# MDFahimAnjum/AliasFree-Diffusion-Models-PyTorch

Hardware: AMD Instinct MI355X
Metric: train_step_images_per_sec (higher is better)
Workload: dtype f32; 1 GPU; CIFAR-10 32x32x3 synthetic, UNet variant=3 (Config D), batch 256/GPU, T=1000, AdamW lr 3e-4, random-init weights (seed 42); global_batch=256, parallelism=dp1, hip_graph=True, launch_mode=lanes

## Files before the change

### aliasfree-diffusion-models-pytorch_amd/_lib.py

```python
import ctypes
import os
import re

_PKG = os.path.dirname(os.path.abspath(__file__))
_ROOT = os.path.dirname(_PKG)
HEADER = os.path.join(_ROOT, "include", "afd.h")
LIBPATH = os.environ.get("AFD_LIBPATH") or os.path.join(_PKG, "libafd_hip.so")

_CTYPES = {
    "int": ctypes.c_int, "long": ctypes.c_long, "float": ctypes.c_float, "double": ctypes.c_double,
    "size_t": ctypes.c_size_t,
}
_DECL = re.compile(r"^(int|size_t|const char\*)\s+(afd_\w+)\s*\(([^;]*?)\)\s*;", re.M | re.S)


def _strip_comments(src):
    return re.sub(r"/\*.*?\*/", " ", src, flags=re.S)


def parse_header(path=HEADER):
    out = {}
    for ret, name, args in _DECL.findall(_strip_comments(open(path).read())):
        argtypes = []
        args = " ".join(args.split())
        if args not in ("", "void"):
            for a in args.split(","):
                a = a.strip()
                if "*" in a or a.startswith("afd_stream_t"):
                    argtypes.append(ctypes.c_void_p)
                else:
                    base = a.split()[0] if not a.startswith("unsigned") else a
                    argtypes.append(_CTYPES[base])
        restype = {"int": ctypes.c_int, "size_t": ctypes.c_size_t, "const char*": ctypes.c_char_p}[ret]
        out[name] = (restype, argtypes)
    return out


_VALUE_RETURNING = {"afd_device_count", "afd_tok_supported", "afd_conv3x3_weight_kinds", "afd_conv_wgrad_form", "afd_conv_wgrad3_plan",
                    "afd_grad_sqnorm_n_partials", "afd_debug_conv_state"}


class AfdError(RuntimeError):
    pass


class _Lib:
    def __init__(self):
        if not os.path.exists(LIBPATH):
            raise AfdError(
                f"{LIBPATH} not found: build it with `python -c 'import __graft_entry__ as g; g.build()'` "
                "(hipcc --offload-arch=gfx950). There is no CPU/eager fallback.")
        self.cdll = ctypes.CDLL(LIBPATH)
        self.sigs = parse_header()
        for name, (restype, argtypes) in self.sigs.items():
# ... 28 lines not shown
```

### aliasfree-diffusion-models-pytorch_amd/csrc/tok.hip

```cpp
#include "tok_common.h"
#include "tok_h2.h"
#include <algorithm>
#include <cstdint>
#include <mutex>
#include <set>

namespace afd {

template <int KB>
__device__ __forceinline__ f32x16 t_block(const float* __restrict__ Ws, int nb, int l31, int half, const TT<KB>& z, f32x16 acc) {
  constexpr int WS = 32 * KB + 4;
  const float* __restrict__ wr = Ws + (nb * 32 + l31) * WS + 4 * half;
#pragma unroll
  for (int j = 0; j < KB; ++j)
#pragma unroll
    for (int q = 0; q < 4; ++q) {
      const float4 a = *reinterpret_cast<const float4*>(wr + 32 * j + 8 * q);
      acc = __builtin_amdgcn_mfma_f32_32x32x2f32(a.x, z.b[j][4 * q + 0], acc, 0, 0, 0);
      acc = __builtin_amdgcn_mfma_f32_32x32x2f32(a.y, z.b[j][4 * q + 1], acc, 0, 0, 0);
      acc = __builtin_amdgcn_mfma_f32_32x32x2f32(a.z, z.b[j][4 * q + 2], acc, 0, 0, 0);
      acc = __builtin_amdgcn_mfma_f32_32x32x2f32(a.w, z.b[j][4 * q + 3], acc, 0, 0, 0);
    }
  return acc;
}
// ... 639 lines not shown
static int g_tok_max_wg = 0;
static int g_tok_path = 0;
static bool use_h2(int C, long ntile, int kern) {
  if (C != 64 && C != 128) return false;
  if (g_tok_path >= 4) return true;
  if (g_tok_path != 0) return false;
  if (C == 64) return ntile >= 1024 || (kern == 2 && ntile >= 512);
  return kern != 1 && ntile >= 512;
}
static bool use_wide(int C, long ntile) {
  if (C != 64 && C != 128) return false;
  if (g_tok_max_wg > 0 || g_tok_path == 1) return false;
  if (g_tok_path == 2) return true;
  return C == 128 || ntile < 1024;
}
static unsigned chain_grid(int C, long ntile) {
  const long wg = (ntile + 3) / 4;
  const long cap = g_tok_max_wg > 0 ? g_tok_max_wg : (C > 64 ? 8192 : 1024);
  return (unsigned)std::min<long>(wg, cap);
}

}

using namespace afd;

extern "C" {

int afd_tok_supported(int C) { return tok_ok(C) ? 1 : 0; }
int afd_debug_tok_grid(int max_workgroups) { g_tok_max_wg = max_workgroups; return AFD_OK; }
int afd_debug_tok_path(int mode) {
  AFD_REQUIRE(mode >= 0 && mode <= 6, "afd_debug_tok_path: mode %d not in 0..6", mode);
  g_tok_path = mode;
  tok_h2_debug_tpw(mode == 5 ? 2 : (mode == 6 ? 4 : 0));
  return AFD_OK;
}

int afd_tok_head_fwd(const float* x, const float* gamma, const float* beta, const float* w, const float* bias, float* h_out,
                     float* stats_out, float* qkv, int B, int C, int P, float eps, afd_stream_t st) {
  AFD_REQUIRE(x && gamma && beta && w && qkv && B > 0 && P > 0, "afd_tok_head_fwd: NULL pointer or empty shape");
  AFD_REQUIRE(tok_ok(C), "afd_tok_head_fwd: C=%d not covered (32, 64, 128)", C);
  AFD_REQUIRE((long)B * P * 3 * C < (1L << 31), "afd_tok_head_fwd: tensor too large for 32-bit offsets");
  const int N = 3 * C;
  const long ntile = ((long)B * P + 31) / 32, wg_tiles = (ntile + 3) / 4;
  if (use_h2(C, ntile, 0)) return tok_h2_head_fwd(x, gamma, beta, w, bias, h_out, stats_out, qkv, B, C, P, eps, g_tok_max_wg, as_stream(st));
  if (use_wide(C, ntile) && aligned16(w) && (ntile <= 256 || g_tok_path == 2)) {
    const long waves = ntile * (N / 32);
    const dim3 wgrid((unsigned)((waves + 3) / 4));
    hipStream_t s = as_stream(st);
    if (C == 64) hipLaunchKernelGGL((tok_head_fwd_wide<64, 1>), wgrid, dim3(256), 0, s, x, gamma, beta, w, bias, h_out, stats_out, qkv, B, P, eps);
    else         hipLaunchKernelGGL((tok_head_fwd_wide<128, 1>), wgrid, dim3(256), 0, s, x, gamma, beta, w, bias, h_out, stats_out, qkv, B, P, eps);
    return check_launch("afd_tok_head_fwd");
  }
  int npw = 32;
  for (int cand : {N, 192, 128, 96, 64, 32}) {
    if (cand > N || N % cand != 0) continue;
    if (sizeof(float) * ((size_t)cand * (C + 5) + 2 * C) > 64 * 1024) continue;
    npw = cand;
    if (wg_tiles * (N / cand) >= 256) break;
  }
  const size_t lds = sizeof(float) * ((size_t)npw * (C + 5) + 2 * C);
// ... 6 lines not shown
  }
  return check_launch("afd_tok_head_fwd");
}

int afd_tok_tail_fwd(const float* att, const float* x, const float* wo, const float* bo, const float* gamma, const float* beta,
                     const float* w1, const float* b1, const float* w2, const float* b2, float* a_out, float* stats_out,
                     float* f_out, float* u_out, float* g_out, float* out, int B, int C, int P, float eps, afd_stream_t st) {
  AFD_REQUIRE(att && x && wo && bo && gamma && beta && w1 && b1 && w2 && b2 && out && B > 0 && P > 0,
              "afd_tok_tail_fwd: NULL pointer or empty shape");
  AFD_REQUIRE(tok_ok(C), "afd_tok_tail_fwd: C=%d not covered (32, 64, 128)", C);
  AFD_REQUIRE((long)B * P * C < (1L << 31), "afd_tok_tail_fwd: tensor too large for 32-bit offsets");
  const bool train = a_out != nullptr;
  AFD_REQUIRE(!train || (stats_out && f_out && u_out && g_out), "afd_tok_tail_fwd: a_out given but a saved-tensor pointer is NULL");
  const long ntile = ((long)B * P + 31) / 32;
  hipStream_t s = as_stream(st);
  if (use_h2(C, ntile, 1))
    return tok_h2_tail_fwd(att, x, wo, bo, gamma, beta, w1, b1, w2, b2, a_out, stats_out, f_out, u_out, g_out, out, B, C, P, eps, g_tok_max_wg, s);
  if (use_wide(C, ntile) && aligned16(wo) && aligned16(w1) && aligned16(w2)) {
    const dim3 wgrid((unsigned)((ntile + Wide<64>::TPW - 1) / Wide<64>::TPW)), wgrid128((unsigned)ntile);
#define AFD_TAILW(C_, T_, G_) hipLaunchKernelGGL((tok_tail_fwd_wide<C_, T_>), G_, dim3(256), 0, s, att, x, wo, bo, gamma, beta, w1, b1, w2, b2, \
                                                  a_out, stats_out, f_out, u_out, g_out, out, B, P, eps)
    if (C == 64) { if (train) AFD_TAILW(64, true, wgrid); else AFD_TAILW(64, false, wgrid); }
    else         { if (train) AFD_TAILW(128, true, wgrid128); else AFD_TAILW(128, false, wgrid128); }
#undef AFD_TAILW
    return check_launch("afd_tok_tail_fwd");
  }
  const size_t lds = chain_lds(C, 5);
  const dim3 grid(chain_grid(C, ntile));
#define AFD_TAIL(C_, T_) do { if (int rc = set_lds(tok_tail_fwd<C_, T_>, lds)) return rc; \
    hipLaunchKernelGGL((tok_tail_fwd<C_, T_>), grid, dim3(256), lds, s, att, x, wo, bo, gamma, beta, w1, b1, w2, b2, a_out, stats_out, \
                       f_out, u_out, g_out, out, B, P, eps); } while (0)
  switch (C) {
    case 32:  if (train) AFD_TAIL(32, true); else AFD_TAIL(32, false); break;
// ... 1 lines not shown
    default:  if (train) AFD_TAIL(128, true); else AFD_TAIL(128, false); break;
  }
#undef AFD_TAIL
  return check_launch("afd_tok_tail_fwd");
}

int afd_tok_tail_bwd(const float* d_out, const float* u, const float* a, const float* stats, const float* gamma, const float* w2,
                     const float* w1, const float* wo, float* du_out, float* df_out, float* da_out, float* datt_out, int B, int C,
                     int P, afd_stream_t st) {
  AFD_REQUIRE(d_out && u && a && stats && gamma && w2 && w1 && wo && du_out && df_out && da_out && datt_out && B > 0 && P > 0,
              "afd_tok_tail_bwd: NULL pointer or empty shape");
  AFD_REQUIRE(tok_ok(C), "afd_tok_tail_bwd: C=%d not covered (32, 64, 128)", C);
  AFD_REQUIRE((long)B * P * C < (1L << 31), "afd_tok_tail_bwd: tensor too large for 32-bit offsets");
  const long ntile = ((long)B * P + 31) / 32;
  hipStream_t s = as_stream(st);
  if (use_h2(C, ntile, 2)) return tok_h2_tail_bwd(d_out, u, a, stats, gamma, w2, w1, wo, du_out, df_out, da_out, datt_out, B, C, P, g_tok_max_wg, s);
  if (use_wide(C, ntile)) {
    if (C == 64) hipLaunchKernelGGL(tok_tail_bwd_wide<64>, dim3((unsigned)((ntile + 1) / 2)), dim3(256), 0, s, d_out, u, a, stats, gamma, w2, w1, wo, du_out, df_out, da_out, datt_out, B, P);
    else         hipLaunchKernelGGL(tok_tail_bwd_wide<128>, dim3((unsigned)ntile), dim3(256), 0, s, d_out, u, a, stats, gamma, w2, w1, wo, du_out, df_out, da_out, datt_out, B, P);
    return check_launch("afd_tok_tail_bwd");
  }
  const size_t lds = chain_lds(C, 1);
  const dim3 grid(chain_grid(C, ntile));
#define AFD_TB(C_) do { if (int rc = set_lds(tok_tail_bwd<C_>, lds)) return rc; \
    hipLaunchKernelGGL(tok_tail_bwd<C_>, grid, dim3(256), lds, s, d_out, u, a, stats, gamma, w2, w1, wo, du_out, df_out, da_out, datt_out, B, P); } while (0)
  switch (C) { case 32: AFD_TB(32); break; case 64: AFD_TB(64); break; default: AFD_TB(128); break; }
#undef AFD_TB
  return check_launch("afd_tok_tail_bwd");
}

int afd_tok_head_bwd(const float* dqkv, const float* x, const float* stats, const float* gamma, const float* w_in,
                     const float* d_res, float* dh_out, float* dx_out, int B, int C, int P, afd_stream_t st) {
  AFD_REQUIRE(dqkv && x && stats && gamma && w_in && d_res && dx_out && B > 0 && P > 0, "afd_tok_head_bwd: NULL pointer or empty shape");
  AFD_REQUIRE(tok_ok(C), "afd_tok_head_bwd: C=%d not covered (32, 64, 128)", C);
  AFD_REQUIRE((long)B * P * 3 * C < (1L << 31), "afd_tok_head_bwd: tensor too large for 32-bit offsets");
  const long ntile = ((long)B * P + 31) / 32;
  hipStream_t s = as_stream(st);
  if (use_h2(C, ntile, 3)) return tok_h2_head_bwd(dqkv, x, stats, gamma, w_in, d_res, dh_out, dx_out, B, C, P, g_tok_max_wg, s);
  if (use_wide(C, ntile)) {
    if (C == 64) hipLaunchKernelGGL(tok_head_bwd_wide<64>, dim3((unsigned)((ntile + 1) / 2)), dim3(256), 0, s, dqkv, x, stats, gamma, w_in, d_res, dh_out, dx_out, B, P);
    else         hipLaunchKernelGGL(tok_head_bwd_wide<128>, dim3((unsigned)ntile), dim3(256), 0, s, dqkv, x, stats, gamma, w_in, d_res, dh_out, dx_out, B, P);
    return check_launch("afd_tok_head_bwd");
  }
  const size_t lds = chain_lds(C, 1);
  const dim3 grid(chain_grid(C, ntile));
#define AFD_HB(C_) do { if (int rc = set_lds(tok_head_bwd<C_>, lds)) return rc; \
    hipLaunchKernelGGL(tok_head_bwd<C_>, grid, dim3(256), lds, s, dqkv, x, stats, gamma, w_in, d_res, dh_out, dx_out, B, P); } while (0)
  switch (C) { case 32: AFD_HB(32); break; case 64: AFD_HB(64); break; default: AFD_HB(128); break; }
#undef AFD_HB
  return check_launch("afd_tok_head_bwd");
}

}
```

### aliasfree-diffusion-models-pytorch_amd/csrc/tok_h2.hip

```cpp
#include "tok_common.h"
#include "h2_common.h"
#include "tok_h2.h"
#include <algorithm>

namespace afd {

template <int NB>
__device__ __forceinline__ void h_load(TT<NB>& z, const float* __restrict__ src, unsigned base, int P) {
#pragma unroll
  for (int j = 0; j < NB; ++j)
#pragma unroll
    for (int r = 0; r < 16; ++r) z.b[j][r] = (src + (size_t)tch(j, r) * P)[base];
}
template <int NB>
__device__ __forceinline__ void h_store(const TT<NB>& z, float* __restrict__ dst, unsigned base, int P, bool live) {
  if (!live) return;
#pragma unroll
  for (int j = 0; j < NB; ++j)
#pragma unroll
    for (int r = 0; r < 16; ++r) (dst + (size_t)tch(j, r) * P)[base] = z.b[j][r];
}

template <int KB> struct HP { h8 a[2 * KB], b[2 * KB]; };

template <int KB>
__device__ __forceinline__ float hp_split(const TT<KB>& z, HP<KB>& p) {
  float m = 0.f;
#pragma unroll
  for (int j = 0; j < KB; ++j)
#pragma unroll
    for (int r = 0; r < 16; ++r) m = fmaxf(m, fabsf(z.b[j][r]));
  m = fmaxf(m, __shfl_xor(m, 32, 64));
  const float s = h2_scale_for(m);
#pragma unroll
  for (int k = 0; k < 2 * KB; ++k) {
    float x[8];
// ... 6 lines not shown

template <int KB>
__device__ __forceinline__ f32x16 hp_block(const h8* __restrict__ img, int nb, int l31, int half, const HP<KB>& z) {
  constexpr int C = 32 * KB, NG = C / 8;
  const h8* __restrict__ w0 = img + half * C + nb * 32 + l31;
  const h8* __restrict__ w1 = w0 + NG * C;
  f32x16 acc = zero16();
#pragma unroll
  for (int k = 0; k < 2 * KB; ++k) {
    const h8 a1 = w0[2 * k * C], a2 = w1[2 * k * C];
    acc = __builtin_amdgcn_mfma_f32_32x32x16_f16(a2, z.a[k], acc, 0, 0, 0);
    acc = __builtin_amdgcn_mfma_f32_32x32x16_f16(a1, z.b[k], acc, 0, 0, 0);
    acc = __builtin_amdgcn_mfma_f32_32x32x16_f16(a1, z.a[k], acc, 0, 0, 0);
  }
  return acc;
}

template <int C> struct H2Lds {
  static constexpr int NG = C / 8, REC = 2 * NG * C;
  static constexpr bool RELOAD = C > 64;
  static constexpr int NSLOT = RELOAD ? 2 : 3;
  h8* img[3];
  float* winv[3];
  unsigned* rmax[3];
  float* vec;
  __device__ __forceinline__ void init(unsigned char* base) {
    h8* i0 = reinterpret_cast<h8*>(base);
    float* w0 = reinterpret_cast<float*>(i0 + NSLOT * REC);
    unsigned* r0 = reinterpret_cast<unsigned*>(w0 + NSLOT * C);
#pragma unroll
    for (int m = 0; m < 3; ++m) {
      const int s = m % NSLOT;
      img[m] = i0 + s * REC; winv[m] = w0 + s * C; rmax[m] = r0 + s * C;
    }
    vec = reinterpret_cast<float*>(r0 + NSLOT * C);
  }
  static size_t bytes(int nvec) { return (size_t)NSLOT * REC * 16 + (size_t)NSLOT * C * 8 + (size_t)nvec * C * 4; }
};

struct WSrc { const float* w; int ldw, n0, k0; };

template <int C, int NT> struct Stg {
  static constexpr int NG = C / 8, NR = C * NG / NT;
  float x[NR][8];
  static __device__ __forceinline__ void rec(int r, bool transposed, int& n, int& G) {
    const int i = (int)threadIdx.x + r * NT;
    if (transposed) { n = i % C; G = i / C; }
    else {
      const int lo = i & 63, hi = i >> 6;
      n = (hi % (C / 8)) * 8 + (lo & 7);
      G = (hi / (C / 8)) * 8 + (lo >> 3);
    }
  }
  __device__ __forceinline__ void load(const WSrc& q, bool transposed) {
#pragma unroll
    for (int r = 0; r < NR; ++r) {
      int n, G;
      rec(r, transposed, n, G);
      const int kb = 16 * (G >> 1) + 4 * (G & 1);
#pragma unroll
      for (int e = 0; e < 8; ++e) {
        const int k = kb + 8 * (e >> 2) + (e & 3);
        x[r][e] = transposed ? q.w[(long)(q.k0 + k) * q.ldw + q.n0 + n] : q.w[(long)(q.n0 + n) * q.ldw + q.k0 + k];
      }
    }
  }
  __device__ __forceinline__ void maxima(unsigned* __restrict__ rmax, bool transposed) const {
#pragma unroll
    for (int r = 0; r < NR; ++r) {
      int n, G;
      rec(r, transposed, n, G);
      float m = 0.f;
#pragma unroll
      for (int e = 0; e < 8; ++e) m = fmaxf(m, fabsf(x[r][e]));
      atomicMax(&rmax[n], __float_as_uint(m));
    }
  }
  __device__ __forceinline__ void store(h8* __restrict__ img, float* __restrict__ winv, const unsigned* __restrict__ rmax,
                                        bool transposed) const {
#pragma unroll
    for (int r = 0; r < NR; ++r) {
      int n, G;
      rec(r, transposed, n, G);
      const float sc = h2_scale_for(__uint_as_float(rmax[n]));
      h8 p0, p1;
      h2_split8(x[r], sc, p0, p1);
      img[G * C + n] = p0;
      img[(NG + G) * C + n] = p1;
      if (G == 0) winv[n] = h2_inv_pow2(sc);
    }
  }
};

template <int C, int NT, int M0, int CNT>
__device__ __forceinline__ void h2_stage(const H2Lds<C>& L, const WSrc* src, bool transposed) {
  Stg<C, NT> st[CNT];
#pragma unroll
  for (int i = 0; i < CNT; ++i) st[i].load(src[i], transposed);
#pragma unroll
  for (int i = 0; i < CNT; ++i)
    for (int c = threadIdx.x; c < C; c += NT) L.rmax[M0 + i][c] = 0u;
  __syncthreads();
#pragma unroll
  for (int i = 0; i < CNT; ++i) st[i].maxima(L.rmax[M0 + i], transposed);
  __syncthreads();
#pragma unroll
  for (int i = 0; i < CNT; ++i) st[i].store(L.img[M0 + i], L.winv[M0 + i], L.rmax[M0 + i], transposed);
  __builtin_amdgcn_sched_barrier(0);
}
template <int C, int NT>
__device__ __forceinline__ void h2_stage_first(const H2Lds<C>& L, const WSrc* src, bool transposed) {
  if (H2Lds<C>::RELOAD) h2_stage<C, NT, 0, 2>(L, src, transposed);
  else h2_stage<C, NT, 0, 3>(L, src, transposed);
}
template <int C, int NT, int M>
__device__ __forceinline__ void h2_stage_one(const H2Lds<C>& L, const WSrc* src, bool transposed) {
  h2_stage<C, NT, M, 1>(L, src + M, transposed);
}

struct Walk { int lane, wv, half, l31, ntile, tstride, t0, npass; unsigned total; };
template <int TPW> __device__ __forceinline__ Walk walk_of(int B, int P) {
  Walk k;
  k.lane = threadIdx.x & 63; k.wv = threadIdx.x >> 6; k.half = k.lane >> 5; k.l31 = k.lane & 31;
  k.total = (unsigned)B * (unsigned)P;
  k.ntile = (int)((k.total + 31u) / 32u);
  k.tstride = gridDim.x * TPW;
  k.t0 = blockIdx.x * TPW;
  k.npass = k.t0 < k.ntile ? (k.ntile - k.t0 + k.tstride - 1) / k.tstride : 0;
  return k;
}

extern __shared__ __attribute__((aligned(16))) unsigned char h2_smem[];
// ... 352 lines not shown
```

### include/afd.h

```cpp
#ifndef AFD_H_
#define AFD_H_

#include <stddef.h>
#include <stdint.h>

#ifdef __cplusplus
extern "C" {
#endif

#define AFD_OK 0
#define AFD_EINVAL 1
#define AFD_ELAUNCH 2
#define AFD_MAX_TAPS 15

typedef void* afd_stream_t;

const char* afd_version(void);
const char* afd_last_error(void);
int afd_device_count(void);

int afd_lowpass_kernel(double omega_c, int N, int has_beta, double beta, float* taps_out);

int afd_filt_up2_fwd(const float* x, float* y, int B, int C, int H, int W, long x_bstride, long y_bstride,
                     const float* taps, int N, afd_stream_t stream);
// ... 88 lines not shown
                        afd_stream_t stream);
int afd_layernorm_c_bwd_params(const float* x, const float* dy, const float* stats, int B, int C, int HW,
                               float* dgamma_dbeta_partial , float* dgamma, float* dbeta, int accumulate,
                               afd_stream_t stream);
int afd_layernorm_c_bwd_partials(const float* x, const float* dy, const float* stats, int B, int C, int HW, float* part,
                                 afd_stream_t stream);

int afd_debug_attn_rows(int rows);
int afd_attn_fwd(const float* qkv, float* o, float* lse, int B, int heads, int d, int L, afd_stream_t stream);
int afd_attn_bwd(const float* qkv, const float* o, const float* d_o, const float* lse, float* dqkv,
                 float* delta_workspace , int B, int heads, int d, int L, afd_stream_t stream);

int afd_tok_supported(int C);
int afd_debug_tok_grid(int max_workgroups);
int afd_debug_tok_path(int mode);
int afd_tok_head_fwd(const float* x, const float* gamma, const float* beta, const float* w_in, const float* b_in,
                     float* h_out, float* stats_out, float* qkv, int B, int C, int P, float eps, afd_stream_t stream);
int afd_tok_tail_fwd(const float* att, const float* x, const float* w_o, const float* b_o, const float* gamma, const float* beta,
                     const float* w_1, const float* b_1, const float* w_2, const float* b_2,
                     float* a_out, float* stats_out, float* f_out, float* u_out, float* g_out, float* out,
                     int B, int C, int P, float eps, afd_stream_t stream);
int afd_tok_tail_bwd(const float* d_out, const float* u, const float* a, const float* stats, const float* gamma,
                     const float* w_2, const float* w_1, const float* w_o,
                     float* du_out, float* df_out, float* da_out, float* datt_out, int B, int C, int P, afd_stream_t stream);
int afd_tok_head_bwd(const float* dqkv, const float* x, const float* stats, const float* gamma, const float* w_in,
                     const float* d_res, float* dh_out, float* dx_out, int B, int C, int P, afd_stream_t stream);

int afd_gelu_fwd(const float* x, float* y, long n, afd_stream_t stream);
int afd_gelu_bwd(const float* x, const float* dy, float* dx, long n, afd_stream_t stream);
int afd_maxpool2_fwd(const float* x, float* y, int B, int C, int H, int W, afd_stream_t stream);
// ... 299 lines not shown
```

Baseline: 39740 images/s.

## Add wide split-half tokenizer kernels for mid-size attention token counts

```diff
diff --git a/aliasfree-diffusion-models-pytorch_amd/_lib.py b/aliasfree-diffusion-models-pytorch_amd/_lib.py
--- a/aliasfree-diffusion-models-pytorch_amd/_lib.py
+++ b/aliasfree-diffusion-models-pytorch_amd/_lib.py
@@ -37,7 +37,7 @@
 
 
 _VALUE_RETURNING = {"afd_device_count", "afd_tok_supported", "afd_conv3x3_weight_kinds", "afd_conv_wgrad_form", "afd_conv_wgrad3_plan",
-                    "afd_grad_sqnorm_n_partials", "afd_debug_conv_state"}
+                    "afd_grad_sqnorm_n_partials", "afd_debug_conv_state", "afd_debug_tok_form"}
 
 
 class AfdError(RuntimeError):
diff --git a/aliasfree-diffusion-models-pytorch_amd/csrc/tok.hip b/aliasfree-diffusion-models-pytorch_amd/csrc/tok.hip
--- a/aliasfree-diffusion-models-pytorch_amd/csrc/tok.hip
+++ b/aliasfree-diffusion-models-pytorch_amd/csrc/tok.hip
@@ -1,5 +1,6 @@
 #include "tok_common.h"
 #include "tok_h2.h"
+#include "tok_h2w.h"
 #include <algorithm>
 #include <cstdint>
 #include <mutex>
@@ -677,6 +678,19 @@
   if (g_tok_path == 2) return true;
   return C == 128 || ntile < 1024;
 }
+static bool use_h2w(int C, long ntile, int kern) {
+  if (C != 64 && C != 128) return false;
+  if (g_tok_path == 7) return true;
+  if (g_tok_path != 0) return false;
+  if (C == 64) return ntile >= 512 && ntile < 1024 && kern != 1;
+  return ntile >= 128 && ntile < 512 && kern >= 2;
+}
+static int tok_form(int C, long ntile, int kern) {
+  if (use_h2w(C, ntile, kern)) return 3;
+  if (use_h2(C, ntile, kern)) return 2;
+  if (use_wide(C, ntile) && (kern != 0 || ntile <= 256 || g_tok_path == 2)) return 1;
+  return 0;
+}
 static unsigned chain_grid(int C, long ntile) {
   const long wg = (ntile + 3) / 4;
   const long cap = g_tok_max_wg > 0 ? g_tok_max_wg : (C > 64 ? 8192 : 1024);
@@ -692,10 +706,14 @@
 int afd_tok_supported(int C) { return tok_ok(C) ? 1 : 0; }
 int afd_debug_tok_grid(int max_workgroups) { g_tok_max_wg = max_workgroups; return AFD_OK; }
 int afd_debug_tok_path(int mode) {
-  AFD_REQUIRE(mode >= 0 && mode <= 6, "afd_debug_tok_path: mode %d not in 0..6", mode);
+  AFD_REQUIRE(mode >= 0 && mode <= 7, "afd_debug_tok_path: mode %d not in 0..7", mode);
   g_tok_path = mode;
   tok_h2_debug_tpw(mode == 5 ? 2 : (mode == 6 ? 4 : 0));
   return AFD_OK;
+}
+int afd_debug_tok_form(int C, int B, int P, int kern) {
+  if (!tok_ok(C) || B <= 0 || P <= 0 || kern < 0 || kern > 3) return -1;
+  return tok_form(C, ((long)B * P + 31) / 32, kern);
 }
 
 int afd_tok_head_fwd(const float* x, const float* gamma, const float* beta, const float* w, const float* bias, float* h_out,
@@ -705,8 +723,10 @@
   AFD_REQUIRE((long)B * P * 3 * C < (1L << 31), "afd_tok_head_fwd: tensor too large for 32-bit offsets");
   const int N = 3 * C;
   const long ntile = ((long)B * P + 31) / 32, wg_tiles = (ntile + 3) / 4;
-  if (use_h2(C, ntile, 0)) return tok_h2_head_fwd(x, gamma, beta, w, bias, h_out, stats_out, qkv, B, C, P, eps, g_tok_max_wg, as_stream(st));
-  if (use_wide(C, ntile) && aligned16(w) && (ntile <= 256 || g_tok_path == 2)) {
+  const int form = tok_form(C, ntile, 0);
+  if (form == 3) return tok_h2w_head_fwd(x, gamma, beta, w, bias, h_out, stats_out, qkv, B, C, P, eps, g_tok_max_wg, as_stream(st));
+  if (form == 2) return tok_h2_head_fwd(x, gamma, beta, w, bias, h_out, stats_out, qkv, B, C, P, eps, g_tok_max_wg, as_stream(st));
+  if (form == 1 && aligned16(w)) {
     const long waves = ntile * (N / 32);
     const dim3 wgrid((unsigned)((waves + 3) / 4));
     hipStream_t s = as_stream(st);
@@ -743,9 +763,12 @@
   AFD_REQUIRE(!train || (stats_out && f_out && u_out && g_out), "afd_tok_tail_fwd: a_out given but a saved-tensor pointer is NULL");
   const long ntile = ((long)B * P + 31) / 32;
   hipStream_t s = as_stream(st);
-  if (use_h2(C, ntile, 1))
+  const int form = tok_form(C, ntile, 1);
+  if (form == 3)
+    return tok_h2w_tail_fwd(att, x, wo, bo, gamma, beta, w1, b1, w2, b2, a_out, stats_out, f_out, u_out, g_out, out, B, C, P, eps, g_tok_max_wg, s);
+  if (form == 2)
     return tok_h2_tail_fwd(att, x, wo, bo, gamma, beta, w1, b1, w2, b2, a_out, stats_out, f_out, u_out, g_out, out, B, C, P, eps, g_tok_max_wg, s);
-  if (use_wide(C, ntile) && aligned16(wo) && aligned16(w1) && aligned16(w2)) {
+  if (form == 1 && aligned16(wo) && aligned16(w1) && aligned16(w2)) {
     const dim3 wgrid((unsigned)((ntile + Wide<64>::TPW - 1) / Wide<64>::TPW)), wgrid128((unsigned)ntile);
 #define AFD_TAILW(C_, T_, G_) hipLaunchKernelGGL((tok_tail_fwd_wide<C_, T_>), G_, dim3(256), 0, s, att, x, wo, bo, gamma, beta, w1, b1, w2, b2, \
                                                   a_out, stats_out, f_out, u_out, g_out, out, B, P, eps)
@@ -777,8 +800,10 @@
   AFD_REQUIRE((long)B * P * C < (1L << 31), "afd_tok_tail_bwd: tensor too large for 32-bit offsets");
   const long ntile = ((long)B * P + 31) / 32;
   hipStream_t s = as_stream(st);
-  if (use_h2(C, ntile, 2)) return tok_h2_tail_bwd(d_out, u, a, stats, gamma, w2, w1, wo, du_out, df_out, da_out, datt_out, B, C, P, g_tok_max_wg, s);
-  if (use_wide(C, ntile)) {
+  const int form = tok_form(C, ntile, 2);
+  if (form == 3) return tok_h2w_tail_bwd(d_out, u, a, stats, gamma, w2, w1, wo, du_out, df_out, da_out, datt_out, B, C, P, g_tok_max_wg, s);
+  if (form == 2) return tok_h2_tail_bwd(d_out, u, a, stats, gamma, w2, w1, wo, du_out, df_out, da_out, datt_out, B, C, P, g_tok_max_wg, s);
+  if (form == 1) {
     if (C == 64) hipLaunchKernelGGL(tok_tail_bwd_wide<64>, dim3((unsigned)((ntile + 1) / 2)), dim3(256), 0, s, d_out, u, a, stats, gamma, w2, w1, wo, du_out, df_out, da_out, datt_out, B, P);
     else         hipLaunchKernelGGL(tok_tail_bwd_wide<128>, dim3((unsigned)ntile), dim3(256), 0, s, d_out, u, a, stats, gamma, w2, w1, wo, du_out, df_out, da_out, datt_out, B, P);
     return check_launch("afd_tok_tail_bwd");
@@ -799,8 +824,10 @@
   AFD_REQUIRE((long)B * P * 3 * C < (1L << 31), "afd_tok_head_bwd: tensor too large for 32-bit offsets");
   const long ntile = ((long)B * P + 31) / 32;
   hipStream_t s = as_stream(st);
-  if (use_h2(C, ntile, 3)) return tok_h2_head_bwd(dqkv, x, stats, gamma, w_in, d_res, dh_out, dx_out, B, C, P, g_tok_max_wg, s);
-  if (use_wide(C, ntile)) {
+  const int form = tok_form(C, ntile, 3);
+  if (form == 3) return tok_h2w_head_bwd(dqkv, x, stats, gamma, w_in, d_res, dh_out, dx_out, B, C, P, g_tok_max_wg, s);
+  if (form == 2) return tok_h2_head_bwd(dqkv, x, stats, gamma, w_in, d_res, dh_out, dx_out, B, C, P, g_tok_max_wg, s);
+  if (form == 1) {
     if (C == 64) hipLaunchKernelGGL(tok_head_bwd_wide<64>, dim3((unsigned)((ntile + 1) / 2)), dim3(256), 0, s, dqkv, x, stats, gamma, w_in, d_res, dh_out, dx_out, B, P);
     else         hipLaunchKernelGGL(tok_head_bwd_wide<128>, dim3((unsigned)ntile), dim3(256), 0, s, dqkv, x, stats, gamma, w_in, d_res, dh_out, dx_out, B, P);
     return check_launch("afd_tok_head_bwd");
diff --git a/aliasfree-diffusion-models-pytorch_amd/csrc/tok_h2.hip b/aliasfree-diffusion-models-pytorch_amd/csrc/tok_h2.hip
--- a/aliasfree-diffusion-models-pytorch_amd/csrc/tok_h2.hip
+++ b/aliasfree-diffusion-models-pytorch_amd/csrc/tok_h2.hip
@@ -1,25 +1,8 @@
-#include "tok_common.h"
-#include "h2_common.h"
+#include "tok_h2_image.h"
 #include "tok_h2.h"
 #include <algorithm>
 
 namespace afd {
-
-template <int NB>
-__device__ __forceinline__ void h_load(TT<NB>& z, const float* __restrict__ src, unsigned base, int P) {
-#pragma unroll
-  for (int j = 0; j < NB; ++j)
-#pragma unroll
-    for (int r = 0; r < 16; ++r) z.b[j][r] = (src + (size_t)tch(j, r) * P)[base];
-}
-template <int NB>
-__device__ __forceinline__ void h_store(const TT<NB>& z, float* __restrict__ dst, unsigned base, int P, bool live) {
-  if (!live) return;
-#pragma unroll
-  for (int j = 0; j < NB; ++j)
-#pragma unroll
-    for (int r = 0; r < 16; ++r) (dst + (size_t)tch(j, r) * P)[base] = z.b[j][r];
-}
 
 template <int KB> struct HP { h8 a[2 * KB], b[2 * KB]; };
 
@@ -56,108 +39,6 @@
     acc = __builtin_amdgcn_mfma_f32_32x32x16_f16(a1, z.a[k], acc, 0, 0, 0);
   }
   return acc;
-}
-
-template <int C> struct H2Lds {
-  static constexpr int NG = C / 8, REC = 2 * NG * C;
-  static constexpr bool RELOAD = C > 64;
-  static constexpr int NSLOT = RELOAD ? 2 : 3;
-  h8* img[3];
-  float* winv[3];
-  unsigned* rmax[3];
-  float* vec;
-  __device__ __forceinline__ void init(unsigned char* base) {
-    h8* i0 = reinterpret_cast<h8*>(base);
-    float* w0 = reinterpret_cast<float*>(i0 + NSLOT * REC);
-    unsigned* r0 = reinterpret_cast<unsigned*>(w0 + NSLOT * C);
-#pragma unroll
-    for (int m = 0; m < 3; ++m) {
-      const int s = m % NSLOT;
-      img[m] = i0 + s * REC; winv[m] = w0 + s * C; rmax[m] = r0 + s * C;
-    }
-    vec = reinterpret_cast<float*>(r0 + NSLOT * C);
-  }
-  static size_t bytes(int nvec) { return (size_t)NSLOT * REC * 16 + (size_t)NSLOT * C * 8 + (size_t)nvec * C * 4; }
-};
-
-struct WSrc { const float* w; int ldw, n0, k0; };
-
-template <int C, int NT> struct Stg {
-  static constexpr int NG = C / 8, NR = C * NG / NT;
-  float x[NR][8];
-  static __device__ __forceinline__ void rec(int r, bool transposed, int& n, int& G) {
-    const int i = (int)threadIdx.x + r * NT;
-    if (transposed) { n = i % C; G = i / C; }
-    else {
-      const int lo = i & 63, hi = i >> 6;
-      n = (hi % (C / 8)) * 8 + (lo & 7);
-      G = (hi / (C / 8)) * 8 + (lo >> 3);
-    }
-  }
-  __device__ __forceinline__ void load(const WSrc& q, bool transposed) {
-#pragma unroll
-    for (int r = 0; r < NR; ++r) {
-      int n, G;
-      rec(r, transposed, n, G);
-      const int kb = 16 * (G >> 1) + 4 * (G & 1);
-#pragma unroll
-      for (int e = 0; e < 8; ++e) {
-        const int k = kb + 8 * (e >> 2) + (e & 3);
-        x[r][e] = transposed ? q.w[(long)(q.k0 + k) * q.ldw + q.n0 + n] : q.w[(long)(q.n0 + n) * q.ldw + q.k0 + k];
-      }
-    }
-  }
-  __device__ __forceinline__ void maxima(unsigned* __restrict__ rmax, bool transposed) const {
-#pragma unroll
-    for (int r = 0; r < NR; ++r) {
-      int n, G;
-      rec(r, transposed, n, G);
-      float m = 0.f;
-#pragma unroll
-      for (int e = 0; e < 8; ++e) m = fmaxf(m, fabsf(x[r][e]));
-      atomicMax(&rmax[n], __float_as_uint(m));
-    }
-  }
-  __device__ __forceinline__ void store(h8* __restrict__ img, float* __restrict__ winv, const unsigned* __restrict__ rmax,
-                                        bool transposed) const {
-#pragma unroll
-    for (int r = 0; r < NR; ++r) {
-      int n, G;
-      rec(r, transposed, n, G);
-      const float sc = h2_scale_for(__uint_as_float(rmax[n]));
-      h8 p0, p1;
-      h2_split8(x[r], sc, p0, p1);
-      img[G * C + n] = p0;
-      img[(NG + G) * C + n] = p1;
-      if (G == 0) winv[n] = h2_inv_pow2(sc);
-    }
-  }
-};
-
-template <int C, int NT, int M0, int CNT>
-__device__ __forceinline__ void h2_stage(const H2Lds<C>& L, const WSrc* src, bool transposed) {
-  Stg<C, NT> st[CNT];
-#pragma unroll
-  for (int i = 0; i < CNT; ++i) st[i].load(src[i], transposed);
-#pragma unroll
-  for (int i = 0; i < CNT; ++i)
-    for (int c = threadIdx.x; c < C; c += NT) L.rmax[M0 + i][c] = 0u;
-  __syncthreads();
-#pragma unroll
-  for (int i = 0; i < CNT; ++i) st[i].maxima(L.rmax[M0 + i], transposed);
-  __syncthreads();
-#pragma unroll
-  for (int i = 0; i < CNT; ++i) st[i].store(L.img[M0 + i], L.winv[M0 + i], L.rmax[M0 + i], transposed);
-  __builtin_amdgcn_sched_barrier(0);
-}
-template <int C, int NT>
-__device__ __forceinline__ void h2_stage_first(const H2Lds<C>& L, const WSrc* src, bool transposed) {
-  if (H2Lds<C>::RELOAD) h2_stage<C, NT, 0, 2>(L, src, transposed);
-  else h2_stage<C, NT, 0, 3>(L, src, transposed);
-}
-template <int C, int NT, int M>
-__device__ __forceinline__ void h2_stage_one(const H2Lds<C>& L, const WSrc* src, bool transposed) {
-  h2_stage<C, NT, M, 1>(L, src + M, transposed);
 }
 
 struct Walk { int lane, wv, half, l31, ntile, tstride, t0, npass; unsigned total; };
diff --git a/aliasfree-diffusion-models-pytorch_amd/csrc/tok_h2_image.h b/aliasfree-diffusion-models-pytorch_amd/csrc/tok_h2_image.h
--- /dev/null
+++ b/aliasfree-diffusion-models-pytorch_amd/csrc/tok_h2_image.h
@@ -0,0 +1,125 @@
+#pragma once
+#include "tok_common.h"
+#include "h2_common.h"
+
+namespace afd {
+
+template <int NB>
+__device__ __forceinline__ void h_load(TT<NB>& z, const float* __restrict__ src, unsigned base, int P) {
+#pragma unroll
+  for (int j = 0; j < NB; ++j)
+#pragma unroll
+    for (int r = 0; r < 16; ++r) z.b[j][r] = (src + (size_t)tch(j, r) * P)[base];
+}
+template <int NB>
+__device__ __forceinline__ void h_store(const TT<NB>& z, float* __restrict__ dst, unsigned base, int P, bool live) {
+  if (!live) return;
+#pragma unroll
+  for (int j = 0; j < NB; ++j)
+#pragma unroll
+    for (int r = 0; r < 16; ++r) (dst + (size_t)tch(j, r) * P)[base] = z.b[j][r];
+}
+
+template <int C> struct H2Lds {
+  static constexpr int NG = C / 8, REC = 2 * NG * C;
+  static constexpr bool RELOAD = C > 64;
+  static constexpr int NSLOT = RELOAD ? 2 : 3;
+  h8* img[3];
+  float* winv[3];
+  unsigned* rmax[3];
+  float* vec;
+  __device__ __forceinline__ void init(unsigned char* base) {
+    h8* i0 = reinterpret_cast<h8*>(base);
+    float* w0 = reinterpret_cast<float*>(i0 + NSLOT * REC);
+    unsigned* r0 = reinterpret_cast<unsigned*>(w0 + NSLOT * C);
+#pragma unroll
+    for (int m = 0; m < 3; ++m) {
+      const int s = m % NSLOT;
+      img[m] = i0 + s * REC; winv[m] = w0 + s * C; rmax[m] = r0 + s * C;
+    }
+    vec = reinterpret_cast<float*>(r0 + NSLOT * C);
+  }
+  static size_t bytes(int nvec) { return (size_t)NSLOT * REC * 16 + (size_t)NSLOT * C * 8 + (size_t)nvec * C * 4; }
+};
+
+struct WSrc { const float* w; int ldw, n0, k0; };
+
+template <int C, int NT> struct Stg {
+  static constexpr int NG = C / 8, NR = C * NG / NT;
+  float x[NR][8];
+  static __device__ __forceinline__ void rec(int r, bool transposed, int& n, int& G) {
+    const int i = (int)threadIdx.x + r * NT;
+    if (transposed) { n = i % C; G = i / C; }
+    else {
+      const int lo = i & 63, hi = i >> 6;
+      n = (hi % (C / 8)) * 8 + (lo & 7);
+      G = (hi / (C / 8)) * 8 + (lo >> 3);
+    }
+  }
+  __device__ __forceinline__ void load(const WSrc& q, bool transposed) {
+#pragma unroll
+    for (int r = 0; r < NR; ++r) {
+      int n, G;
+      rec(r, transposed, n, G);
+      const int kb = 16 * (G >> 1) + 4 * (G & 1);
+#pragma unroll
+      for (int e = 0; e < 8; ++e) {
+        const int k = kb + 8 * (e >> 2) + (e & 3);
+        x[r][e] = transposed ? q.w[(long)(q.k0 + k) * q.ldw + q.n0 + n] : q.w[(long)(q.n0 + n) * q.ldw + q.k0 + k];
+      }
+    }
+  }
+  __device__ __forceinline__ void maxima(unsigned* __restrict__ rmax, bool transposed) const {
+#pragma unroll
+    for (int r = 0; r < NR; ++r) {
+      int n, G;
+      rec(r, transposed, n, G);
+      float m = 0.f;
+#pragma unroll
+      for (int e = 0; e < 8; ++e) m = fmaxf(m, fabsf(x[r][e]));
+      atomicMax(&rmax[n], __float_as_uint(m));
+    }
+  }
+  __device__ __forceinline__ void store(h8* __restrict__ img, float* __restrict__ winv, const unsigned* __restrict__ rmax,
+                                        bool transposed) const {
+#pragma unroll
+    for (int r = 0; r < NR; ++r) {
+      int n, G;
+      rec(r, transposed, n, G);
+      const float sc = h2_scale_for(__uint_as_float(rmax[n]));
+      h8 p0, p1;
+      h2_split8(x[r], sc, p0, p1);
+      img[G * C + n] = p0;
+      img[(NG + G) * C + n] = p1;
+      if (G == 0) winv[n] = h2_inv_pow2(sc);
+    }
+  }
+};
+
+template <int C, int NT, int M0, int CNT>
+__device__ __forceinline__ void h2_stage(const H2Lds<C>& L, const WSrc* src, bool transposed) {
+  Stg<C, NT> st[CNT];
+#pragma unroll
+  for (int i = 0; i < CNT; ++i) st[i].load(src[i], transposed);
+#pragma unroll
+  for (int i = 0; i < CNT; ++i)
+    for (int c = threadIdx.x; c < C; c += NT) L.rmax[M0 + i][c] = 0u;
+  __syncthreads();
+#pragma unroll
+  for (int i = 0; i < CNT; ++i) st[i].maxima(L.rmax[M0 + i], transposed);
+  __syncthreads();
+#pragma unroll
+  for (int i = 0; i < CNT; ++i) st[i].store(L.img[M0 + i], L.winv[M0 + i], L.rmax[M0 + i], transposed);
+  __builtin_amdgcn_sched_barrier(0);
+}
+template <int C, int NT>
+__device__ __forceinline__ void h2_stage_first(const H2Lds<C>& L, const WSrc* src, bool transposed) {
+  if (H2Lds<C>::RELOAD) h2_stage<C, NT, 0, 2>(L, src, transposed);
+  else h2_stage<C, NT, 0, 3>(L, src, transposed);
+}
+template <int C, int NT, int M>
+__device__ __forceinline__ void h2_stage_one(const H2Lds<C>& L, const WSrc* src, bool transposed) {
+  h2_stage<C, NT, M, 1>(L, src + M, transposed);
+}
+
+}
diff --git a/aliasfree-diffusion-models-pytorch_amd/csrc/tok_h2w.h b/aliasfree-diffusion-models-pytorch_amd/csrc/tok_h2w.h
--- /dev/null
+++ b/aliasfree-diffusion-models-pytorch_amd/csrc/tok_h2w.h
@@ -0,0 +1,17 @@
+#pragma once
+#include "common.h"
+
+namespace afd {
+
+int tok_h2w_head_fwd(const float* x, const float* gamma, const float* beta, const float* w, const float* bias, float* h_out,
+                     float* stats_out, float* qkv, int B, int C, int P, float eps, int max_wg, hipStream_t s);
+int tok_h2w_tail_fwd(const float* att, const float* x, const float* wo, const float* bo, const float* gamma, const float* beta,
+                     const float* w1, const float* b1, const float* w2, const float* b2, float* a_out, float* stats_out,
+                     float* f_out, float* u_out, float* g_out, float* out, int B, int C, int P, float eps, int max_wg, hipStream_t s);
+int tok_h2w_tail_bwd(const float* d_out, const float* u, const float* a, const float* stats, const float* gamma, const float* w2,
+                     const float* w1, const float* wo, float* du_out, float* df_out, float* da_out, float* datt_out, int B, int C,
+                     int P, int max_wg, hipStream_t s);
+int tok_h2w_head_bwd(const float* dqkv, const float* x, const float* stats, const float* gamma, const float* w_in,
+                     const float* d_res, float* dh_out, float* dx_out, int B, int C, int P, int max_wg, hipStream_t s);
+
+}
diff --git a/aliasfree-diffusion-models-pytorch_amd/csrc/tok_h2w.hip b/aliasfree-diffusion-models-pytorch_amd/csrc/tok_h2w.hip
--- /dev/null
+++ b/aliasfree-diffusion-models-pytorch_amd/csrc/tok_h2w.hip
@@ -0,0 +1,441 @@
+#include "tok_h2_image.h"
+#include "tok_h2w.h"
+#include <algorithm>
+
+namespace afd {
+
+constexpr int kWSlots = 6;
+
+template <int C> struct WTile {
+  static constexpr int KB = C / 32, NG = C / 8, OPREC = 2 * NG * 32;
+  h8* op;
+  float* xs;
+  int j, l31, half;
+  __device__ __forceinline__ void init(float* after_vec, int TG, int tg, int j_, int l31_, int half_) {
+    h8* o0 = reinterpret_cast<h8*>(after_vec);
+    op = o0 + tg * OPREC;
+    xs = reinterpret_cast<float*>(o0 + TG * OPREC) + tg * (kWSlots * KB * 32);
+    j = j_; l31 = l31_; half = half_;
+  }
+  static size_t bytes(int TG) { return (size_t)TG * ((size_t)OPREC * 16 + (size_t)kWSlots * KB * 32 * 4); }
+
+  template <int SLOT> __device__ __forceinline__ float sum(float v) const {
+    float* a = xs + SLOT * KB * 32;
+    if (half == 0) a[j * 32 + l31] = v;
+    __syncthreads();
+    float s = a[l31];
+#pragma unroll
+    for (int w = 1; w < KB; ++w) s += a[w * 32 + l31];
+    return s;
+  }
+  template <int SLOT> __device__ __forceinline__ void sum2(float& v0, float& v1) const {
+    float* a = xs + SLOT * KB * 32;
+    float* b = a + KB * 32;
+    if (half == 0) { a[j * 32 + l31] = v0; b[j * 32 + l31] = v1; }
+    __syncthreads();
+    float s0 = a[l31], s1 = b[l31];
+#pragma unroll
+    for (int w = 1; w < KB; ++w) { s0 += a[w * 32 + l31]; s1 += b[w * 32 + l31]; }
+    v0 = s0; v1 = s1;
+  }
+  template <int SLOT> __device__ __forceinline__ float feed(const f32x16& z) const {
+    float m = 0.f;
+#pragma unroll
+    for (int r = 0; r < 16; ++r) m = fmaxf(m, fabsf(z[r]));
+    m = fmaxf(m, __shfl_xor(m, 32, 64));
+    float* a = xs + SLOT * KB * 32;
+    if (half == 0) a[j * 32 + l31] = m;
+    __syncthreads();
+    m = a[l31];
+#pragma unroll
+    for (int w = 1; w < KB; ++w) m = fmaxf(m, a[w * 32 + l31]);
+    const float s = h2_scale_for(m);
+#pragma unroll
+    for (int q = 0; q < 2; ++q) {
+      float x[8];
+#pragma unroll
+      for (int e = 0; e < 8; ++e) x[e] = z[8 * q + e];
+      h8 p0, p1;
+      h2_split8(x, s, p0, p1);
+      const int G = 2 * (2 * j + q) + half;
+      op[G * 32 + l31] = p0;
+      op[(NG + G) * 32 + l31] = p1;
+    }
+    __syncthreads();
+    return h2_inv_pow2(s);
+  }
+  __device__ __forceinline__ f32x16 block(const h8* __restrict__ img) const {
+    const h8* __restrict__ w0 = img + half * C + j * 32 + l31;
+    const h8* __restrict__ w1 = w0 + NG * C;
+    const h8* __restrict__ z0 = op + half * 32 + l31;
+    const h8* __restrict__ z1 = z0 + NG * 32;
+    f32x16 acc = zero16();
+#pragma unroll
+    for (int k = 0; k < 2 * KB; ++k) {
+      const h8 a1 = w0[2 * k * C], a2 = w1[2 * k * C];
+      const h8 b1 = z0[2 * k * 32], b2 = z1[2 * k * 32];
+      acc = __builtin_amdgcn_mfma_f32_32x32x16_f16(a2, b1, acc, 0, 0, 0);
+      acc = __builtin_amdgcn_mfma_f32_32x32x16_f16(a1, b2, acc, 0, 0, 0);
+      acc = __builtin_amdgcn_mfma_f32_32x32x16_f16(a1, b1, acc, 0, 0, 0);
+    }
+    return acc;
+  }
+  template <int SLOT> __device__ __forceinline__ void ln_fwd(const f32x16& x, const float* __restrict__ gs, const float* __restrict__ bs,
+                                                             float eps, f32x16& y, float& mean, float& rstd) const {
+    constexpr float invC = 1.0f / C;
+    float s = 0.f;
+#pragma unroll
+    for (int r = 0; r < 16; ++r) s += x[r];
+    s += __shfl_xor(s, 32, 64);
+    mean = sum<SLOT>(s) * invC;
+    float q = 0.f;
+#pragma unroll
+    for (int r = 0; r < 16; ++r) { const float d = x[r] - mean; q = fmaf(d, d, q); }
+    q += __shfl_xor(q, 32, 64);
+    rstd = 1.0f / sqrtf(sum<SLOT + 1>(q) * invC + eps);
+#pragma unroll
+    for (int r = 0; r < 16; ++r) {
+      const int c = tch(0, r) + 4 * half;
+      y[r] = (x[r] - mean) * rstd * gs[32 * j + c] + bs[32 * j + c];
+    }
+  }
+  template <int SLOT> __device__ __forceinline__ void ln_bwd(f32x16& dy, const f32x16& x, const float* __restrict__ gs, float mean,
+                                                             float rstd, const f32x16& add) const {
+    constexpr float invC = 1.0f / C;
+    float s1 = 0.f, s2 = 0.f;
+#pragma unroll
+    for (int r = 0; r < 16; ++r) {
+      const float gv = gs[32 * j + tch(0, r) + 4 * half] * dy[r];
+      const float xh = (x[r] - mean) * rstd;
+      dy[r] = gv;
+      s1 += gv;
+      s2 = fmaf(gv, xh, s2);
+    }
+    s1 += __shfl_xor(s1, 32, 64);
+    s2 += __shfl_xor(s2, 32, 64);
+    sum2<SLOT>(s1, s2);
+    const float m1 = s1 * invC, m2 = s2 * invC;
+#pragma unroll
+    for (int r = 0; r < 16; ++r) {
+      const float xh = (x[r] - mean) * rstd;
+      dy[r] = rstd * (dy[r] - m1 - xh * m2) + add[r];
+    }
+  }
+};
+
+__device__ __forceinline__ f32x16 wb_load(const float* __restrict__ src, int j, unsigned base, int P) {
+  TT<1> z;
+  h_load(z, src + (size_t)(32 * j) * P, base, P);
+  return z.b[0];
+}
+__device__ __forceinline__ void wb_store(const f32x16& v, float* __restrict__ dst, int j, unsigned base, int P, bool live) {
+  TT<1> z;
+  z.b[0] = v;
+  h_store(z, dst + (size_t)(32 * j) * P, base, P, live);
+}
+
+struct WWalk { int j, tg, half, l31, ntile, tstride, t0, npass; unsigned total; };
+template <int KB, int TG> __device__ __forceinline__ WWalk wwalk_of(int B, int P) {
+  WWalk k;
+  const int lane = threadIdx.x & 63, wv = __builtin_amdgcn_readfirstlane((int)(threadIdx.x >> 6));
+  k.j = wv % KB; k.tg = wv / KB; k.half = lane >> 5; k.l31 = lane & 31;
+  k.total = (unsigned)B * (unsigned)P;
+  k.ntile = (int)((k.total + 31u) / 32u);
+  k.tstride = gridDim.x * TG;
+  k.t0 = blockIdx.x * TG;
+  k.npass = k.t0 < k.ntile ? (k.ntile - k.t0 + k.tstride - 1) / k.tstride : 0;
+  return k;
+}
+__device__ __forceinline__ Pix wpix(const WWalk& k, int pass, int P) {
+  const int t = k.t0 + k.tg + pass * k.tstride;
+  const bool active = t < k.ntile;
+  Pix pc = pix_of(active ? t : 0, k.l31, k.total, P);
+  pc.live = pc.live && active;
+  return pc;
+}
+
+extern __shared__ __attribute__((aligned(16))) unsigned char h2w_smem[];
+
+template <int C, int TG>
+__global__ __launch_bounds__(2 * C * TG) void tok_h2w_head_fwd_k(const float* __restrict__ x, const float* __restrict__ gamma,
+                                                                  const float* __restrict__ beta, const float* __restrict__ w,
+                                                                  const float* __restrict__ bias, float* __restrict__ h_out,
+                                                                  float* __restrict__ stats_out, float* __restrict__ y, int B, int P,
+                                                                  float eps) {
+  using LD = H2Lds<C>;
+  constexpr int KB = C / 32, NT = 64 * KB * TG;
+  LD L;
+  L.init(h2w_smem);
+  float* vec = L.vec;
+  const WWalk k = wwalk_of<KB, TG>(B, P);
+  WTile<C> T;
+  T.init(vec + 5 * C, TG, k.tg, k.j, k.l31, k.half);
+  const int half = k.half, j = k.j;
+  const WSrc src[3] = {{w, C, 0, 0}, {w, C, C, 0}, {w, C, 2 * C, 0}};
+  h2_stage_first<C, NT>(L, src, false);
+  for (int i = threadIdx.x; i < C; i += NT) { vec[i] = gamma[i]; vec[C + i] = beta[i]; }
+  for (int i = threadIdx.x; i < 3 * C; i += NT) vec[2 * C + i] = bias ? bias[i] : 0.f;
+  for (int pass = 0; pass < k.npass; ++pass) {
+    __syncthreads();
+    if (LD::RELOAD && pass > 0) { h2_stage_one<C, NT, 0>(L, src, false); __syncthreads(); }
+    const Pix pc = wpix(k, pass, P);
+    const unsigned base = tbase(pc, C, P, half), yb = tbase(pc, 3 * C, P, half);
+    const f32x16 xc = wb_load(x, j, base, P);
+    f32x16 h;
+    float mean, rstd;
+    T.template ln_fwd<0>(xc, vec, vec + C, eps, h, mean, rstd);
+    if (h_out) wb_store(h, h_out, j, base, P, pc.live);
+    if (stats_out && pc.live && half == 0 && j == 0) { stats_out[2 * pc.f] = mean; stats_out[2 * pc.f + 1] = rstd; }
+    const float is = T.template feed<2>(h);
+#pragma unroll
+    for (int sl = 0; sl < 3; ++sl) {
+      if (LD::RELOAD && sl == 1) { __syncthreads(); h2_stage_one<C, NT, 2>(L, src, false); }
+      if (LD::RELOAD && sl == 2) __syncthreads();
+      const f32x16 acc = T.block(L.img[sl]);
+      if (pc.live) {
+#pragma unroll
+        for (int r = 0; r < 16; ++r) {
+          const int c = j * 32 + tch(0, r) + 4 * half;
+          (y + (size_t)(sl * C + j * 32 + tch(0, r)) * P)[yb] = acc[r] * is * L.winv[sl][c] + vec[2 * C + sl * C + c];
+        }
+      }
+    }
+  }
+}
+
+template <int C, int TG, bool TRAIN>
+__global__ __launch_bounds__(2 * C * TG) void tok_h2w_tail_fwd_k(const float* __restrict__ att, const float* __restrict__ xres,
+                                                                  const float* __restrict__ wo, const float* __restrict__ bo,
+                                                                  const float* __restrict__ gamma, const float* __restrict__ beta,
+                                                                  const float* __restrict__ w1, const float* __restrict__ b1,
+                                                                  const float* __restrict__ w2, const float* __restrict__ b2,
+                                                                  float* __restrict__ a_out, float* __restrict__ stats_out,
+                                                                  float* __restrict__ f_out, float* __restrict__ u_out,
+                                                                  float* __restrict__ g_out, float* __restrict__ out, int B, int P,
+                                                                  float eps) {
+  using LD = H2Lds<C>;
+  constexpr int KB = C / 32, NT = 64 * KB * TG;
+  LD L;
+  L.init(h2w_smem);
+  float* vec = L.vec;
+  const WWalk k = wwalk_of<KB, TG>(B, P);
+  WTile<C> T;
+  T.init(vec + 5 * C, TG, k.tg, k.j, k.l31, k.half);
+  const int half = k.half, j = k.j;
+  const WSrc src[3] = {{wo, C, 0, 0}, {w1, C, 0, 0}, {w2, C, 0, 0}};
+  h2_stage_first<C, NT>(L, src, false);
+  for (int i = threadIdx.x; i < C; i += NT) {
+    vec[i] = bo[i]; vec[C + i] = gamma[i]; vec[2 * C + i] = beta[i]; vec[3 * C + i] = b1[i]; vec[4 * C + i] = b2[i];
+  }
+  for (int pass = 0; pass < k.npass; ++pass) {
+    __syncthreads();
+    if (LD::RELOAD && pass > 0) { h2_stage_one<C, NT, 0>(L, src, false); __syncthreads(); }
+    const Pix pc = wpix(k, pass, P);
+    const unsigned base = tbase(pc, C, P, half);
+    const f32x16 z = wb_load(att, j, base, P), xr = wb_load(xres, j, base, P);
+    float is = T.template feed<0>(z);
+    f32x16 acc = T.block(L.img[0]);
+    f32x16 a, f;
+#pragma unroll
+    for (int r = 0; r < 16; ++r) {
+      const int c = j * 32 + tch(0, r) + 4 * half;
+      a[r] = acc[r] * is * L.winv[0][c] + vec[c] + xr[r];
+    }
+    float mean, rstd;
+    T.template ln_fwd<1>(a, vec + C, vec + 2 * C, eps, f, mean, rstd);
+    if (TRAIN) {
+      wb_store(a, a_out, j, base, P, pc.live);
+      wb_store(f, f_out, j, base, P, pc.live);
+      if (pc.live && half == 0 && j == 0) { stats_out[2 * pc.f] = mean; stats_out[2 * pc.f + 1] = rstd; }
+    }
+    is = T.template feed<3>(f);
+    if (LD::RELOAD) h2_stage_one<C, NT, 2>(L, src, false);
+    acc = T.block(L.img[1]);
+    f32x16 u, g;
+#pragma unroll
+    for (int r = 0; r < 16; ++r) {
+      const int c = j * 32 + tch(0, r) + 4 * half;
+      u[r] = acc[r] * is * L.winv[1][c] + vec[3 * C + c];
+      g[r] = gelu_erf(u[r]);
+    }
+    if (TRAIN) {
+      wb_store(u, u_out, j, base, P, pc.live);
+      wb_store(g, g_out, j, base, P, pc.live);
+    }
+    is = T.template feed<4>(g);
+    acc = T.block(L.img[2]);
+    if (pc.live) {
+#pragma unroll
+      for (int r = 0; r < 16; ++r) {
+        const int c = j * 32 + tch(0, r) + 4 * half;
+        (out + (size_t)(j * 32 + tch(0, r)) * P)[base] = acc[r] * is * L.winv[2][c] + vec[4 * C + c] + a[r];
+      }
+    }
+  }
+}
+
+template <int C, int TG>
+__global__ __launch_bounds__(2 * C * TG) void tok_h2w_tail_bwd_k(const float* __restrict__ dout, const float* __restrict__ u_in,
+                                                                  const float* __restrict__ a_in, const float* __restrict__ stats,
+                                                                  const float* __restrict__ gamma, const float* __restrict__ w2,
+                                                                  const float* __restrict__ w1, const float* __restrict__ wo,
+                                                                  float* __restrict__ du_out, float* __restrict__ df_out,
+                                                                  float* __restrict__ da_out, float* __restrict__ datt_out, int B,
+                                                                  int P) {
+  using LD = H2Lds<C>;
+  constexpr int KB = C / 32, NT = 64 * KB * TG;
+  LD L;
+  L.init(h2w_smem);
+  float* gs = L.vec;
+  const WWalk k = wwalk_of<KB, TG>(B, P);
+  WTile<C> T;
+  T.init(gs + C, TG, k.tg, k.j, k.l31, k.half);
+  const int half = k.half, j = k.j;
+  const WSrc src[3] = {{w2, C, 0, 0}, {w1, C, 0, 0}, {wo, C, 0, 0}};
+  h2_stage_first<C, NT>(L, src, true);
+  for (int i = threadIdx.x; i < C; i += NT) gs[i] = gamma[i];
+  for (int pass = 0; pass < k.npass; ++pass) {
+    __syncthreads();
+    if (LD::RELOAD && pass > 0) { h2_stage_one<C, NT, 0>(L, src, true); __syncthreads(); }
+    const Pix pc = wpix(k, pass, P);
+    const unsigned base = tbase(pc, C, P, half);
+    const f32x16 dd = wb_load(dout, j, base, P), uu = wb_load(u_in, j, base, P);
+    float is = T.template feed<0>(dd);
+    f32x16 acc = T.block(L.img[0]);
+    f32x16 du;
+#pragma unroll
+    for (int r = 0; r < 16; ++r) du[r] = acc[r] * is * L.winv[0][j * 32 + tch(0, r) + 4 * half] * gelu_erf_grad(uu[r]);
+    wb_store(du, du_out, j, base, P, pc.live);
+    is = T.template feed<1>(du);
+    if (LD::RELOAD) h2_stage_one<C, NT, 2>(L, src, true);
+    acc = T.block(L.img[1]);
+    f32x16 df;
+#pragma unroll
+    for (int r = 0; r < 16; ++r) df[r] = acc[r] * is * L.winv[1][j * 32 + tch(0, r) + 4 * half];
+    wb_store(df, df_out, j, base, P, pc.live);
+    const f32x16 aa = wb_load(a_in, j, base, P);
+    const float mean = pc.live ? stats[2 * pc.f] : 0.f, rstd = pc.live ? stats[2 * pc.f + 1] : 0.f;
+    T.template ln_bwd<2>(df, aa, gs, mean, rstd, dd);
+    wb_store(df, da_out, j, base, P, pc.live);
+    is = T.template feed<4>(df);
+    acc = T.block(L.img[2]);
+    if (pc.live) {
+#pragma unroll
+      for (int r = 0; r < 16; ++r)
+        (datt_out + (size_t)(j * 32 + tch(0, r)) * P)[base] = acc[r] * is * L.winv[2][j * 32 + tch(0, r) + 4 * half];
+    }
+  }
+}
+
+template <int C, int TG>
+__global__ __launch_bounds__(2 * C * TG) void tok_h2w_head_bwd_k(const float* __restrict__ dqkv, const float* __restrict__ x,
+                                                                  const float* __restrict__ stats, const float* __restrict__ gamma,
+                                                                  const float* __restrict__ w_in, const float* __restrict__ dres,
+                                                                  float* __restrict__ dh_out, float* __restrict__ dx_out, int B,
+                                                                  int P) {
+  using LD = H2Lds<C>;
+  constexpr int KB = C / 32, NT = 64 * KB * TG;
+  LD L;
+  L.init(h2w_smem);
+  float* gs = L.vec;
+  const WWalk k = wwalk_of<KB, TG>(B, P);
+  WTile<C> T;
+  T.init(gs + C, TG, k.tg, k.j, k.l31, k.half);
+  const int half = k.half, j = k.j;
+  const WSrc src[3] = {{w_in, C, 0, 0}, {w_in, C, 0, C}, {w_in, C, 0, 2 * C}};
+  h2_stage_first<C, NT>(L, src, true);
+  for (int i = threadIdx.x; i < C; i += NT) gs[i] = gamma[i];
+  for (int pass = 0; pass < k.npass; ++pass) {
+    __syncthreads();
+    if (LD::RELOAD && pass > 0) { h2_stage_one<C, NT, 0>(L, src, true); __syncthreads(); }
+    const Pix pc = wpix(k, pass, P);
+    const unsigned base = tbase(pc, C, P, half), qb = tbase(pc, 3 * C, P, half);
+    f32x16 dh;
+    {
+      const f32x16 z = wb_load(dqkv, j, qb, P);
+      const float is = T.template feed<0>(z);
+      const f32x16 acc = T.block(L.img[0]);
+#pragma unroll
+      for (int r = 0; r < 16; ++r) dh[r] = acc[r] * is * L.winv[0][j * 32 + tch(0, r) + 4 * half];
+    }
+    {
+      const f32x16 z = wb_load(dqkv + (size_t)C * P, j, qb, P);
+      const float is = T.template feed<1>(z);
+      if (LD::RELOAD) h2_stage_one<C, NT, 2>(L, src, true);
+      const f32x16 acc = T.block(L.img[1]);
+#pragma unroll
+      for (int r = 0; r < 16; ++r) dh[r] += acc[r] * is * L.winv[1][j * 32 + tch(0, r) + 4 * half];
+    }
+    {
+      const f32x16 z = wb_load(dqkv + (size_t)(2 * C) * P, j, qb, P);
+      const float is = T.template feed<2>(z);
+      const f32x16 acc = T.block(L.img[2]);
+#pragma unroll
+      for (int r = 0; r < 16; ++r) dh[r] += acc[r] * is * L.winv[2][j * 32 + tch(0, r) + 4 * half];
+    }
+    if (dh_out) wb_store(dh, dh_out, j, base, P, pc.live);
+    const f32x16 xx = wb_load(x, j, base, P), rr = wb_load(dres, j, base, P);
+    const float mean = pc.live ? stats[2 * pc.f] : 0.f, rstd = pc.live ? stats[2 * pc.f + 1] : 0.f;
+    T.template ln_bwd<3>(dh, xx, gs, mean, rstd, rr);
+    wb_store(dh, dx_out, j, base, P, pc.live);
+  }
+}
+
+static unsigned h2w_grid(int C, long ntile, int tg, int max_wg) {
+  const long wg = (ntile + tg - 1) / tg;
+  const long cap = max_wg > 0 ? max_wg : (C > 64 ? 256 : 512);
+  return (unsigned)std::min<long>(wg, cap);
+}
+
+#define AFD_H2W_LAUNCH(KERN, NVEC, ...)                                                                             \
+  do {                                                                                                              \
+    const size_t lds = H2Lds<KC>::bytes(NVEC) + WTile<KC>::bytes(KG);                                               \
+    if (int rc = lds_opt_in(KERN, lds)) return rc;                                                                  \
+    hipLaunchKernelGGL(KERN, dim3(h2w_grid(KC, ntile, KG, max_wg)), dim3(2 * KC * KG), lds, s, __VA_ARGS__);        \
+  } while (0)
+#define AFD_H2W_SWITCH(BODY)                                                                                        \
+  do {                                                                                                              \
+    if (C == 64) { constexpr int KC = 64, KG = 2; BODY; }                                                           \
+    else         { constexpr int KC = 128, KG = 1; BODY; }                                                          \
+  } while (0)
+
+int tok_h2w_head_fwd(const float* x, const float* gamma, const float* beta, const float* w, const float* bias, float* h_out,
+                     float* stats_out, float* qkv, int B, int C, int P, float eps, int max_wg, hipStream_t s) {
+  const long ntile = ((long)B * P + 31) / 32;
+  AFD_H2W_SWITCH(AFD_H2W_LAUNCH((tok_h2w_head_fwd_k<KC, KG>), 5, x, gamma, beta, w, bias, h_out, stats_out, qkv, B, P, eps));
+  return check_launch("afd_tok_head_fwd");
+}
+
+int tok_h2w_tail_fwd(const float* att, const float* x, const float* wo, const float* bo, const float* gamma, const float* beta,
+                     const float* w1, const float* b1, const float* w2, const float* b2, float* a_out, float* stats_out,
+                     float* f_out, float* u_out, float* g_out, float* out, int B, int C, int P, float eps, int max_wg, hipStream_t s) {
+  const long ntile = ((long)B * P + 31) / 32;
+  if (a_out)
+    AFD_H2W_SWITCH(AFD_H2W_LAUNCH((tok_h2w_tail_fwd_k<KC, KG, true>), 5, att, x, wo, bo, gamma, beta, w1, b1, w2, b2, a_out, stats_out,
+                                  f_out, u_out, g_out, out, B, P, eps));
+  else
+    AFD_H2W_SWITCH(AFD_H2W_LAUNCH((tok_h2w_tail_fwd_k<KC, KG, false>), 5, att, x, wo, bo, gamma, beta, w1, b1, w2, b2, a_out, stats_out,
+                                  f_out, u_out, g_out, out, B, P, eps));
+  return check_launch("afd_tok_tail_fwd");
+}
+
+int tok_h2w_tail_bwd(const float* d_out, const float* u, const float* a, const float* stats, const float* gamma, const float* w2,
+                     const float* w1, const float* wo, float* du_out, float* df_out, float* da_out, float* datt_out, int B, int C,
+                     int P, int max_wg, hipStream_t s) {
+  const long ntile = ((long)B * P + 31) / 32;
+  AFD_H2W_SWITCH(AFD_H2W_LAUNCH((tok_h2w_tail_bwd_k<KC, KG>), 1, d_out, u, a, stats, gamma, w2, w1, wo, du_out, df_out, da_out, datt_out,
+                                B, P));
+  return check_launch("afd_tok_tail_bwd");
+}
+
+int tok_h2w_head_bwd(const float* dqkv, const float* x, const float* stats, const float* gamma, const float* w_in,
+                     const float* d_res, float* dh_out, float* dx_out, int B, int C, int P, int max_wg, hipStream_t s) {
+  const long ntile = ((long)B * P + 31) / 32;
+  AFD_H2W_SWITCH(AFD_H2W_LAUNCH((tok_h2w_head_bwd_k<KC, KG>), 1, dqkv, x, stats, gamma, w_in, d_res, dh_out, dx_out, B, P));
+  return check_launch("afd_tok_head_bwd");
+}
+
+#undef AFD_H2W_SWITCH
+#undef AFD_H2W_LAUNCH
+
+}
diff --git a/include/afd.h b/include/afd.h
--- a/include/afd.h
+++ b/include/afd.h
@@ -126,6 +126,7 @@
 int afd_tok_supported(int C);
 int afd_debug_tok_grid(int max_workgroups);
 int afd_debug_tok_path(int mode);
+int afd_debug_tok_form(int C, int B, int P, int kern);
 int afd_tok_head_fwd(const float* x, const float* gamma, const float* beta, const float* w_in, const float* b_in,
                      float* h_out, float* stats_out, float* qkv, int B, int C, int P, float eps, afd_stream_t stream);
 int afd_tok_tail_fwd(const float* att, const float* x, const float* w_o, const float* b_o, const float* gamma, const float* beta,
```

Result: no change. 39800 images/s (median of 6 runs) (+0.2%).
